# yyNoBug/VAE_segmentation

Measured on AMD Instinct MI355X. Metric: 3D train-step volumes/sec at 96^3 batch=2 (joint VAE+seg), higher is better.
Workload: dtype bf16; 1 GPU; configs[1]: 96^3 joint VAE+seg training step (joint_train), batch=2/GPU, bf16 activations + fp32 accumulate, SGD momentum 0.9, VAE frozen, HIP-graph replay; global_batch=2, parallelism=dp1, activation_recomputation=False, tail_in_graph=True, nranks=1, grad_exchange=none (1 rank)

## Files before the change

include/vaeseg.h:

```cpp
#ifndef VAESEG_H
#define VAESEG_H
#include <stddef.h>
#include <stdint.h>

#ifdef __cplusplus
extern "C" {
#endif

#define VS_VERSION 500

enum { VS_F32 = 0, VS_BF16 = 1, VS_F16 = 2, VS_F32X3 = 3  };
#ifndef VS_STAT_SLOTS
#define VS_STAT_SLOTS 4
#endif
enum { VS_OK = 0, VS_EINVAL = -1, VS_ESHAPE = -2, VS_EDTYPE = -3, VS_EWORKSPACE = -4, VS_EALIGN = -5 };

enum {
    VS_CONV_K3 = 0,
    VS_CONV_K2S2 = 1,
    VS_CONV_T2S2 = 2,
    VS_WGRAD_SLABS = 16,
    VS_CONV_UP = 3
};

enum {
    VS_PACK_ROWS_D0 = 0,
    VS_PACK_ROWS_D1_FLIP = 1,
    VS_PACK_SCATTER_D1 = 2
};

int vs_version(void);
int vs_stat_slots(void);
int vs_stat_interleaved(void);
const char* vs_strerror(int code);
int vs_get_deterministic(void);

int vs_up_supported(int cin, int cm, int co, int dtype);
int vs_up_compose_sizes(int cin, int cm, int co, size_t* out6);
int vs_up_compose(const float* w2, const float* b2, const float* w3, float* weff, void* img_fwd, void* img_bwd, int* taps_fwd, int* taps_bwd,
                  float* btab, int cin, int cm, int co, int dtype, void* stream);
int vs_up_conv_fwd(const void* x, const double* x_stats, const void* img_fwd, const int* taps_fwd, const float* btab, void* y, double* y_stats,
                   int n, int d, int h, int w, int cin, int co, int dtype, float eps, void* stream);
int vs_up_faces(const void* gy, double* G, int n, int fd, int fh, int fw, int co, int dtype, void* stream);
int vs_up_chain(const float* dweff27, const double* G, const float* w2, const float* b2, const float* w3, float* dw2, float* db2, float* dw3,
                int cin, int cm, int co, void* stream);
int vs_up_conv_bwd_data(const void* gy, const void* img_bwd, const int* taps_bwd, void* gx, const void* mask_x, const double* mask_stats,
                        double* sums, int n, int d, int h, int w, int co, int cin, int dtype, float eps, void* stream);

size_t vs_packed_weight_bytes(int rows, int c_pad, int ntaps, int dtype);
int vs_pack_weight(const float* src, void* dst, int d0, int d1, int ntaps, int c_pad, int form, int dtype, void* stream);

typedef struct vs_pack_desc {
    const float* src;
    void* dst;
    int d0, d1, ntaps, c_pad, form, dtype;
    int first_block;
    int pad_;
    long long total;
} vs_pack_desc;
int vs_pack_weight_multi(const vs_pack_desc* descs, int n_desc, int total_blocks, void* stream);

int vs_conv_gather_fwd(const void* x, const double* x_stats, const void* w_packed, const float* bias,
                       void* y, double* y_stats, int n, int d, int h, int w, int c_in, int m_out,
                       int kind, int dtype, float eps, void* stream);

int vs_conv_scatter_fwd(const void* x, const double* x_stats, const void* w_packed, const float* bias,
                        void* y, int n, int d, int h, int w, int c_in, int m_out, int dtype, float eps, void* stream);

int vs_conv_gather_bwd_data(const void* x, const void* w_packed, void* y, const void* mask_x, const double* mask_stats,
                            double* sums, int n, int d, int h, int w, int c_in, int m_out, int kind, int dtype, float eps,
                            void* stream);
int vs_conv_scatter_bwd_data(const void* x, const void* w_packed, void* y, const void* mask_x, const double* mask_stats,
                             double* sums, int n, int d, int h, int w, int c_in, int m_out, int dtype, float eps, void* stream);
int vs_conv_k3_fused_apply_supported(int n, int d, int h, int w, int c_in, int m_out, int lazy_input, int dtype);
int vs_conv_k3_bwd_data_wgrad_supported(int n, int d, int h, int w, int c_in, int m_out, int dtype);
int vs_conv_k3_bwd_data_wgrad_slabs(int n, int d, int h, int w);
int vs_conv_k3_bwd_data_wgrad(const void* g, const void* act_x, const double* act_stats, const double* act_sums, const void* w_packed, void* y,
                              const void* mask_x, const double* mask_stats, double* sums, float* slabs, int n, int d, int h, int w, int c_in,
                              int m_out, int dtype, float eps, void* stream);
int vs_conv_k3_softmax2_bwd_data(const float* prob, const float* gprob, const void* gprob_cl, const void* w_packed, void* y, const void* mask_x,
                                 const double* mask_stats, double* sums, float* slabs, double* bias_part, int n, int d, int h, int w, int dtype,
                                 float eps, float drop_p, unsigned long long drop_seed, void* stream);
typedef struct vs_config {
    int k3_small;
    int k3_tall;
    int k3_wgs_per_cu;
    int k3t_wgs_per_cu;
    int k3f_min_wgs;
    int mt_min_wgs;
    int f32_limbs;
    int g1_limbs;
    int k3x_ck;
    int k3x_toeplitz;
    int fuse_wgrad;
    int epilogue_apply;
    int chain;
    int k2s2_stream;
    int k2s8_wgs_per_cu;
    int up_wgs_per_cu;
    int up_rb;
    int wgrad_uber;
    int wgrad_mpack;
    int wgrad_swap;
    int wgrad_big;
    int wgrad_xcd;
    int k3_short_tiles;
    int wgrad_bias_fold;
    long long wgrad_wgs;
    long long wgrad_f32_tiles;
    long long wgrad_group_wgs;
    long long wgrad_big_min_voxels;
} vs_config;
int vs_config_bytes(void);
int vs_config_from_env(vs_config* c);
int vs_get_config(vs_config* out);
int vs_set_config(const vs_config* cfg);
int vs_conv_k3_bwd_data_applied_supported(int n, int d, int h, int w, int c_in, int m_out, int dtype);
int vs_conv_k3_bwd_data_applied(const void* x, const void* w_packed, void* y, const void* mask_x, const double* mask_stats, double* sums,
                                unsigned int* sync, unsigned int* fault, int n, int d, int h, int w, int c_in, int m_out, int dtype, float eps, void* stream);
int vs_conv_s2_bwd_data_applied_supported(int n, int d, int h, int w, int c_in, int m_out, int scatter, int dtype);
int vs_conv_s2_bwd_data_applied(const void* x, const void* w_packed, void* y, const void* mask_x, const double* mask_stats, double* sums, const void* add,
                                unsigned int* sync, unsigned int* fault, int n, int d, int h, int w, int c_in, int m_out, int scatter, int dtype, float eps,
                                void* stream);
typedef struct vs_chain_layer {
    const void* x;
    const double* x_stats;
    const void* w_packed;
    void* y;
    double* y_stats;
    const void* mask_x;
    const double* mask_stats;
    double* sums;
    int c_in, m_out;
    int apply;
    int reserved_;
} vs_chain_layer;
int vs_conv_k3_chain_supported(int n, int d, int h, int w, int c_max, int dtype);
long long vs_conv_k3_chain_sync_bytes(int n);
int vs_conv_k3_chain(const vs_chain_layer* layers, int n_layers, int backward, const void* add, unsigned int* sync, unsigned int* fault,
                     int n, int d, int h, int w, int dtype, float eps, void* stream);
int vs_conv_k3_f32_limbs(int d, int h, int w, int c_in);

int vs_conv_k3_bwd_data_fused_apply(const void* g, const void* act_x, const double* act_stats, const double* act_sums,
                                    const void* w_packed, void* y, const void* mask_x, const double* mask_stats, double* sums,
                                    void* dx_out, int n, int d, int h, int w, int c_in, int m_out, int dtype, float eps, void* stream);

int vs_conv_k3_softmax2_fwd(const void* x, const double* x_stats, const void* w_packed, const float* bias,
                            float* prob, int n, int d, int h, int w, int c_in, int dtype, float eps, void* stream);
int vs_conv_k3_softmax2_dropout_fwd(const void* x, const double* x_stats, const void* w_packed, const float* bias,
                                    float* prob, int n, int d, int h, int w, int c_in, int dtype, float eps, float drop_p,
                                    unsigned long long drop_seed, void* stream);
int vs_conv_k3_softmax2_cl_fwd(const void* x, const double* x_stats, const void* w_packed, const float* bias,
                               float* prob, void* prob_cl, int n, int d, int h, int w, int c_in, int dtype, float eps, float drop_p,
                               unsigned long long drop_seed, void* stream);

size_t vs_conv_wgrad_workspace_bytes(int n, int dp, int hp, int wp, int m_ch, int c_ch, int kind);
int vs_conv_wgrad(const void* p, const double* p_stats, const void* q, const double* q_stats, float* dw,
                  void* workspace, size_t workspace_bytes, int n, int dp, int hp, int wp, int m_ch, int c_ch,
                  int m_real, int c_real, int kind, int dtype, float eps, void* stream);
typedef struct vs_wgrad_desc {
    const void* p; const double* p_stats;
    const void* q; const double* q_stats;
    float* dw;
    const void* bias_g; float* db;
    long long bias_rows;
// ... 165 lines not shown
```

vae_segmentation_amd/modules.py:

```python
import torch
import torch.nn as nn

from . import ops

_DEFAULT_DTYPE = torch.float32


def set_default_kernel_dtype(dtype):
    global _DEFAULT_DTYPE
    if dtype not in ops.KERNEL_DTYPES:
        raise TypeError("kernel dtype must be torch.float32, torch.bfloat16 or torch.float16")
    _DEFAULT_DTYPE = dtype


def set_kernel_dtype(module, dtype):
    if dtype not in ops.KERNEL_DTYPES:
        raise TypeError("kernel dtype must be torch.float32, torch.bfloat16 or torch.float16")
    for m in module.modules():
        if hasattr(m, "kernel_dtype"):
            m.kernel_dtype = dtype
    return module


class Act:
# ... 217 lines not shown
        self.down4 = Down(f[3], f[4], norm_type=norm_type, soft=False)
        self.down5 = Down(f[4], f[5], norm_type=norm_type, soft=False)
        self.side = spatial // 32
        self.top_ch = f[5]
        flat = f[5] * self.side ** 3
        self.fc_mean = nn.Linear(flat, dim)
        self.fc_std = nn.Linear(flat, dim)
        self.fc2 = nn.Linear(dim, flat)
        self.up1 = Up(f[5], f[4], norm_type=norm_type, soft=False)
        self.up2 = Up(f[4], f[3], norm_type=norm_type, soft=False)
        self.up3 = Up(f[3], f[2], norm_type=norm_type, soft=False)
        self.up4 = Up(f[2], f[1], norm_type=norm_type, soft=False)
        self.up5 = Up(f[1], f[0], norm_type=norm_type, soft=False)
        self.out_block = nn.Conv3d(f[0], n_class, 3, padding=1)
        self.final = nn.Softmax(dim=1)
        self.n_class = n_class
        self.spatial = spatial
        self.kernel_dtype = _DEFAULT_DTYPE

    def forward(self, x, if_random=False, scale=1, mid_input=False, dropout=0.0, noise=None):
        ops._require_cuda(x)
        if not mid_input:
            if x.shape[-1] != self.spatial:
                raise ValueError("VAE built for spatial=%d got input side %d" % (self.spatial, x.shape[-1]))
            ops.stats_arena_begin(x.device)
            a = Act(ops.planar_input(x, self.kernel_dtype), None)
            a = self.in_block(a)
            if a.stats is not None:
                ops.mark_defer_apply(a.raw, self.in_block.conv[0])
            for blk in (self.down1, self.down2, self.down3, self.down4, self.down5):
                a = _run_block(blk, a)
                if blk is not self.down5 and a.stats is not None:
                    ops.mark_defer_apply(a.raw, blk.conv[1].conv[6])
            feat = ops.Materialize.apply(a.raw, a.stats, None, None)
            x_mean, x_std = ops.LinearCLPair.apply(feat, self.fc_mean.weight, self.fc_mean.bias, False,
                                                   self.fc_std.weight, self.fc_std.bias, True)
            if if_random:
                if noise is None:
                    noise = torch.randn(x_mean.shape, device=x_mean.device, dtype=torch.float32)
                z = ops.Reparam.apply(x_mean, x_std, noise.to(x_mean.device, torch.float32).contiguous(), scale)
            else:
                z = x_mean
        else:
            ops.stats_arena_begin(x.device)
            z = x
        h = ops.LinearToCL.apply(z, self.fc2.weight, self.fc2.bias, self.top_ch, self.side, self.kernel_dtype)
        a = Act(h, None)
        for blk in (self.up1, self.up2, self.up3, self.up4, self.up5):
            a = _dropout(_run_block(blk, a), dropout)
            if a.stats is not None:
                ops.mark_defer_apply(a.raw, blk.conv[1].conv[6])
        recon = ops.ConvK3Softmax.apply(a.raw, a.stats, self.out_block.weight, self.out_block.bias)
        if not mid_input:
            return recon, x_mean, x_std
        return recon


class Segmentation(nn.Module):

    def __init__(self, n_channels, n_class, norm_type=2, n_fmaps=[8, 16, 32, 64, 128, 256]):
        super().__init__()
        _check_n_class(n_class)
        f = list(n_fmaps)
        self.in_block = Conv(n_channels, f[0], norm_type=norm_type, soft=False)
        self.down1 = Down(f[0], f[1], norm_type=norm_type, soft=False)
        self.down2 = Down(f[1], f[2], norm_type=norm_type, soft=False)
        self.down3 = Down(f[2], f[3], norm_type=norm_type, soft=False)
        self.down4 = Down(f[3], f[4], norm_type=norm_type, soft=False)
        self.up2 = Up(f[4], f[3], norm_type=norm_type, soft=False)
        self.up3 = Up(f[3], f[2], norm_type=norm_type, soft=False)
        self.up4 = Up(f[2], f[1], norm_type=norm_type, soft=False)
        self.up5 = Up(f[1], f[0], norm_type=norm_type, soft=False)
        self.out_block = nn.Conv3d(f[0], n_class, 3, padding=1)
        self.final = nn.Softmax(dim=1)
        self.n_class = n_class
        self.kernel_dtype = _DEFAULT_DTYPE

    def forward(self, data_dict, in_key, out_key, dropout=0.0):
        x = data_dict[in_key]
        ops._require_cuda(x)
        if any(s % 16 for s in x.shape[2:]):
            raise ValueError("Segmentation needs spatial sizes that are multiples of 16, got %s" % (tuple(x.shape[2:]),))
        ops.stats_arena_begin(x.device)
        a = Act(ops.PackPlanar.apply(x, self.kernel_dtype), None)
        x1 = self.in_block(a)
        x2 = _run_block(self.down1, x1)
        x3 = _run_block(self.down2, x2)
        x4 = _run_block(self.down3, x3)
        x5 = _run_block(self.down4, x4)
        u = _dropout(_run_block(self.up2, x5), dropout)
        u = _run_block(self.up3, u)
        u = _dropout(Act(ops.Materialize.apply(u.raw, u.stats, x3.raw, x3.stats, True), None), dropout)
        u = _run_block(self.up4, u)
        u = _dropout(Act(ops.Materialize.apply(u.raw, u.stats, x2.raw, x2.stats, True), None), dropout)
        u = _dropout(_run_block(self.up5, u), dropout)
        if u.stats is not None:
            ops.mark_defer_apply(u.raw, self.up5.conv[1].conv[6])
        if dropout:
            data_dict[out_key] = ops.out_block_softmax(u.raw, u.stats, self.out_block.weight, self.out_block.bias,
                                                       float(dropout), ops.next_dropout_seed())
        else:
            data_dict[out_key] = ops.out_block_softmax(u.raw, u.stats, self.out_block.weight, self.out_block.bias)
        return data_dict


class Joint(nn.Module):

    def __init__(self, models, vae_forward_scale=0.0, vae_decoder_dropout=0.0, seg_dropout=0.0):
        super().__init__()
        self.Seg = models[0]
        self.Vae = models[1]
        self.vae_forward_scale = vae_forward_scale
        self.vae_decoder_dropout = vae_decoder_dropout
        self.seg_dropout = seg_dropout

    def forward(self, data_dict, in_key, out_key, out_key_recon, dropout=False):
        with ops.arena_scope(data_dict[in_key].device):
            if dropout:
                data_dict = self.Seg(data_dict, in_key, out_key, dropout=self.seg_dropout)
                data_dict[out_key_recon], _, _ = self.Vae(data_dict[out_key], if_random=False, scale=self.vae_forward_scale,
                                                          dropout=self.vae_decoder_dropout)
            else:
                data_dict = self.Seg(data_dict, in_key, out_key)
                data_dict[out_key_recon], data_dict["mean"], data_dict["std"] = self.Vae(
                    data_dict[out_key], if_random=False, scale=self.vae_forward_scale)
        return data_dict


def _linear(x2d, fc, relu):
    return ops.LinearCL.apply(x2d.contiguous().view(x2d.shape[0], 1, 1, 1, x2d.shape[1]), fc.weight, fc.bias, relu)


class Encoder(nn.Module):

    def __init__(self, n_channels, dim, norm_type=2, n_fmaps=[8, 16, 32, 64, 128, 256], soft=False, spatial=128):
        super().__init__()
        if spatial % 32 or spatial < 64:
            raise ValueError("spatial must be a multiple of 32 and >= 64")
        f = list(n_fmaps)
        self.in_block = Conv(n_channels, f[0], norm_type=norm_type, soft=False)
        self.down1 = Down(f[0], f[1], norm_type=norm_type, soft=False)
        self.down2 = Down(f[1], f[2], norm_type=norm_type, soft=False)
        self.down3 = Down(f[2], f[3], norm_type=norm_type, soft=False)
        self.down4 = Down(f[3], f[4], norm_type=norm_type, soft=False)
        self.down5 = Down(f[4], f[5], norm_type=norm_type, soft=False)
        self.fc1 = nn.Linear(f[5] * (spatial // 32) ** 3, 1024)
        self.fc2 = nn.Linear(1024, 128)
        self.fc_mean = nn.Linear(128, dim)
        self.spatial = spatial
        self.kernel_dtype = _DEFAULT_DTYPE

    def forward(self, x):
        ops._require_cuda(x)
        if x.shape[-1] != self.spatial:
            raise ValueError("Encoder built for spatial=%d got input side %d" % (self.spatial, x.shape[-1]))
        ops.stats_arena_begin(x.device)
        a = Act(ops.PackPlanar.apply(x.contiguous(), self.kernel_dtype), None)
        a = self.in_block(a)
        for blk in (self.down1, self.down2, self.down3, self.down4, self.down5):
            a = blk(a)
        feat = ops.Materialize.apply(a.raw, a.stats, None, None)
        h = ops.LinearCL.apply(feat, self.fc1.weight, self.fc1.bias, True)
        h = _linear(h, self.fc2, True)
        return torch.sigmoid(_linear(h, self.fc_mean, False))


class Fusion(nn.Module):

# ... 86 lines not shown
```

vae_segmentation_amd/ops.py:

```python
import ctypes as _ctypes
import os
import weakref as _weakref

import torch

from . import _lib
from ._lib import (VS_BF16, VS_CONV_K2S2, VS_CONV_K3, VS_CONV_UP, VS_F16, VS_F32, VS_PACK_ROWS_D0, VS_PACK_ROWS_D1_FLIP,
                   VS_PACK_SCATTER_D1, check, lib)

_DT_TORCH = {VS_F32: torch.float32, VS_BF16: torch.bfloat16, VS_F16: torch.float16}
_DT_VS = {v: k for k, v in _DT_TORCH.items()}
KERNEL_DTYPES = tuple(_DT_VS)
VS_F32X3 = 3
F32X3 = "f32x3"
_DT_TORCH[VS_F32X3] = F32X3
_DT_VS[F32X3] = VS_F32X3
_F32_LIMBS = bool(lib.vs_conv_k3_f32_limbs(96, 96, 96, 8))


def k3_pack_dtype(x):
    if x.dtype == torch.float32 and lib.vs_conv_k3_f32_limbs(x.shape[1], x.shape[2], x.shape[3], x.shape[4]):
        return F32X3
    return x.dtype

# ... 876 lines not shown
    tname = _tname(x)
    with _timed("in_relu_bwd_reduce_kernel<%s>" % tname, 2 * x.numel() * _esize(x), 4.0 * x.numel(), str(tuple(x.shape))):
        check(lib.vs_instnorm_relu_bwd_reduce(g.data_ptr(), x.data_ptr(), xs.data_ptr(), sums.data_ptr(), n, voxels, c, dt,
                                              EPS_IN, _stream()), "instnorm_relu_bwd_reduce")
    gx = g if inplace else torch.empty_like(g)
    with _timed("in_relu_bwd_apply_kernel<%s>" % tname, 3 * x.numel() * _esize(x), 6.0 * x.numel(), str(tuple(x.shape))):
        check(lib.vs_instnorm_relu_bwd_apply(g.data_ptr(), x.data_ptr(), xs.data_ptr(), sums.data_ptr(), gx.data_ptr(), n,
                                             voxels, c, dt, EPS_IN, _stream()), "instnorm_relu_bwd_apply")
    return gx


def _contig(t):
    return t if t.is_contiguous() else t.contiguous()


class ConvK3(torch.autograd.Function):

    @staticmethod
    def forward(ctx, x, xs, weight, bias, live_bias=False):
        _require_cuda(x, weight)
        cout, cin = weight.shape[0], weight.shape[1]
        wp = pack_weight_cached(weight, VS_PACK_ROWS_D0, x.shape[-1], k3_pack_dtype(x))
        ctx.live_bias = bool(live_bias) and bias is not None
        b_use = bias if ctx.live_bias else None
        if b_use is not None and cout < cpad(cout):
            b_use = torch.nn.functional.pad(b_use.detach().float(), (0, cpad(cout) - cout))
        y, ys = conv_gather(x, xs, wp, b_use, cpad(cout), VS_CONV_K3, True, real_channels=(cin, cout))
        ctx.save_for_backward(x, xs, weight)
        ctx.has_bias = bias is not None
        ctx.bias_ref = bias
        ctx.defer = bool(getattr(x, "_vs_defer_apply", False)) and xs is not None
        if ctx.needs_input_grad[2]:
            _count_use(weight)
        ctx.mark_non_differentiable(ys)
        ctx.set_materialize_grads(False)
        return y, ys

    @staticmethod
    def backward(ctx, gy, _gys):
        x, xs, weight = ctx.saved_tensors
        if gy is None:
            return None, None, None, None, None
        gy = _contig(gy)
        cout, cin = weight.shape[0], weight.shape[1]
        gx = gw = gb = None
        lazy = _take_lazy(gy)
        if lazy is not None and not (ctx.needs_input_grad[0] and _fa_supported(gy, x, xs is not None)):
            gy, lazy = apply_lazy(gy, lazy), None
        if ctx.needs_input_grad[0]:
            wpb = pack_weight_cached(weight, VS_PACK_ROWS_D1_FLIP, gy.shape[-1], k3_pack_dtype(gy))
            want_gb0 = ctx.has_bias and ctx.needs_input_grad[3] and ctx.live_bias
            if xs is not None and ctx.needs_input_grad[2] and not want_gb0 and _wgrad_fusable(gy, x, weight):
                gx, gw = conv_bwd_data_lazy(gy, wpb, x, xs, VS_CONV_K3, real_channels=(cout, cin), defer=ctx.defer, lazy=lazy,
                                            fuse_wgrad=(weight, cout, cin))
                gb = _dead_bias_grad(ctx.bias_ref, ctx.bias_ref.shape[0], x.device) if ctx.has_bias and ctx.needs_input_grad[3] else None
                return gx, None, gw, gb, None
            if lazy is not None and xs is not None:
                gx, gy = conv_bwd_data_lazy(gy, wpb, x, xs, VS_CONV_K3, real_channels=(cout, cin), defer=ctx.defer, lazy=lazy,
                                            want_dx=ctx.needs_input_grad[2])
            elif lazy is not None:
                ax, axs, asums = lazy
                gx = torch.empty_like(x)
                dx = torch.empty_like(gy) if ctx.needs_input_grad[2] else None
                n_, d_, h_, w_, c_ = gy.shape
                check(lib.vs_conv_k3_bwd_data_fused_apply(gy.data_ptr(), ax.data_ptr(), axs.data_ptr(), asums.data_ptr(), wpb.data_ptr(), gx.data_ptr(),
                                                          None, None, None, _p(dx), n_, d_, h_, w_, c_, x.shape[-1], vs_dtype(x), EPS_IN, _stream()),
                      "conv_k3_bwd_data_fused_apply")
                gy = dx
            elif xs is not None:
                gx = conv_bwd_data_lazy(gy, wpb, x, xs, VS_CONV_K3, real_channels=(cout, cin), defer=ctx.defer)
            else:
                gx, _ = conv_gather(gy, None, wpb, None, x.shape[-1], VS_CONV_K3, False, real_channels=(cout, cin))
        want_gb = ctx.has_bias and ctx.needs_input_grad[3]
        if ctx.needs_input_grad[2]:
            gw, gb = _side_grads(weight, (gy, x, xs), (gy, None, x, xs, cout, cin, VS_CONV_K3),
                                 (gy, cout) if want_gb and ctx.live_bias else None, ctx.bias_ref if ctx.live_bias else None)
        elif want_gb and ctx.live_bias:
            gb = bias_grad(gy, cout)
        if want_gb and not ctx.live_bias:
            gb = _dead_bias_grad(ctx.bias_ref, ctx.bias_ref.shape[0], x.device)
        return gx, None, gw, gb, None


CHAIN = os.environ.get("VS_CHAIN", "1") != "0"


class ChainLayer(_ct.Structure):
    _fields_ = [("x", _ct.c_void_p), ("x_stats", _ct.c_void_p), ("w_packed", _ct.c_void_p), ("y", _ct.c_void_p), ("y_stats", _ct.c_void_p),
                ("mask_x", _ct.c_void_p), ("mask_stats", _ct.c_void_p), ("sums", _ct.c_void_p), ("c_in", _ct.c_int), ("m_out", _ct.c_int),
                ("apply", _ct.c_int), ("reserved_", _ct.c_int)]


_CHAIN_FAULT = {}


def _chain_fault_word(device):
    key = torch.device(device)
    t = _CHAIN_FAULT.get(key)
    if t is None:
        if torch.cuda.is_current_stream_capturing():
            raise RuntimeError("the chain fault word must exist before a capture starts: run the step eagerly once (GraphedStep warms up)")
        t = _CHAIN_FAULT[key] = torch.zeros(32, dtype=torch.int32, device=key)
    return t


def chain_fault():
    for dev, t in _CHAIN_FAULT.items():
        if int(t[0].item()) != 0:
            raise _lib.VaesegError("a chain kernel on %s gave up a bounded wait (workgroups of one sample not co-resident): results invalid; set VS_CHAIN=0" % (dev,))


def device_is_shared(shared=True):
    global CHAIN, EPILOGUE_APPLY
    on = 0 if shared else 1
    set_config(chain=on, epilogue_apply=on)
    CHAIN = EPILOGUE_APPLY = not shared


def _chain_sync(n, device):
    cnt = lib.vs_conv_k3_chain_sync_bytes(n) // 8
    buf = _new_stats(1, cnt + 16, device, width=1).view(-1)
    off = ((-buf.data_ptr()) % 128) // 8
    return buf[off:off + cnt]


def chain_ok(x, xs, convs):
    if not CHAIN or len(convs) < 2 or len(convs) > 3 or x.dtype not in KERNEL_DTYPES:
        return False
    if getattr(x, "_vs_defer_apply", False):
        return False
    if any(tuple(c.weight.shape[2:]) != (3, 3, 3) for c in convs):
        return False
    n, d, h, w, c = x.shape
    cmax = max([c] + [cpad(cv.weight.shape[0]) for cv in convs])
    return bool(lib.vs_conv_k3_chain_supported(n, d, h, w, cmax, vs_dtype(x)))


class ConvK3Chain(torch.autograd.Function):

    @staticmethod
    def forward(ctx, x, xs, *params):
        _require_cuda(x)
        nl = len(params) // 2
        weights, biases = params[0::2], params[1::2]
        n, d, h, w, _ = x.shape
        layers = (ChainLayer * nl)()
        cur, curs, outs, keep = x, xs, [], []
        nb = fl = 0.0
        for l in range(nl):
            wt = weights[l]
            m = cpad(wt.shape[0])
            wp = pack_weight_cached(wt, VS_PACK_ROWS_D0, cur.shape[-1], k3_pack_dtype(cur))
            y = torch.empty((n, d, h, w, m), dtype=x.dtype, device=x.device)
            ys = _new_stats(n, m, x.device)
            layers[l] = ChainLayer(cur.data_ptr(), _p(curs), wp.data_ptr(), y.data_ptr(), ys.data_ptr(), None, None, None, cur.shape[-1], m, 0, 0)
            keep.append(wp)
            nb += (cur.numel() + y.numel() + wt.numel()) * _esize(x)
            fl += 2.0 * n * d * h * w * 27 * wt.shape[0] * wt.shape[1]
            outs.append((y, ys))
            cur, curs = y, ys
            if ctx.needs_input_grad[2 + 2 * l]:
                _count_use(wt)
        sync = _chain_sync(n, x.device)
        with _timed("k3_chain<%s,fwd,%d>" % (_tname(x), nl), nb, fl, "x%s" % (tuple(x.shape),)):
            check(lib.vs_conv_k3_chain(_ct.addressof(layers), nl, 0, None, sync.data_ptr(), _chain_fault_word(x.device).data_ptr(), n, d, h, w,
                                       vs_dtype(x), EPS_IN, _stream()), "conv_k3_chain (forward)")
# ... 1277 lines not shown
```

vae_segmentation_amd/profiling.py:

```python
import torch

from . import ops

LAST_LAUNCHES = []
HBM_PEAK_GBS = 8000.0
MFMA_PEAK_TFLOPS = {"bf16": 2500.0, "fp16": 2500.0, "f32": 2500.0 / 6.0}


LAST_EVENT_OVERHEAD_US = 0.0


def _spin(us, stream):
    from tools import probe
    probe.check(probe.lib.vs_spin(int(us), stream), "spin")


ops.PROFILE_SPIN[0] = _spin


def event_bracket_overhead_us(trials=24, spin_us=20):
    stream = torch.cuda.current_stream().cuda_stream
    over = []
    for _ in range(trials):
        _spin(ops.PROFILE_PRIME_US, stream)
# ... 8 lines not shown


def collect(fwd_bwd, params, steps=2):
    for p in params:
        p.grad = None
    fwd_bwd()
    torch.cuda.synchronize()
    ops.PROFILE = []
    try:
        for _ in range(steps):
            for p in params:
                p.grad = None
            fwd_bwd()
        torch.cuda.synchronize()
        recs = ops.PROFILE
    finally:
        ops.PROFILE = None
    agg = {}
    global LAST_LAUNCHES, LAST_EVENT_OVERHEAD_US
    LAST_EVENT_OVERHEAD_US = event_bracket_overhead_us()
    dur = lambda e0, e1: max(e0.elapsed_time(e1) - LAST_EVENT_OVERHEAD_US * 1e-3, 1e-4)
    LAST_LAUNCHES = sorted(((dur(e0, e1), kid, det, nb, fl) for kid, nb, fl, det, e0, e1 in recs), reverse=True)
    for kid, nb, fl, det, e0, e1 in recs:
        a = agg.setdefault(kid, {"launches": 0, "ms": 0.0, "bytes": 0.0, "flops": 0.0})
        a["launches"] += 1
        a["ms"] += dur(e0, e1)
        a["bytes"] += nb
        a["flops"] += fl
    for a in agg.values():
        for k in ("launches", "ms", "bytes", "flops"):
            a[k] = a[k] / steps
    return agg


def sources_sha():
    import glob
    import hashlib
    import os
    root = os.path.dirname(os.path.dirname(os.path.abspath(__file__)))
    h = hashlib.sha256()
    files = sorted(glob.glob(os.path.join(root, "vae_segmentation_amd", "csrc", "*.hip")) + glob.glob(os.path.join(root, "vae_segmentation_amd", "csrc", "*.h")) +
                   glob.glob(os.path.join(root, "vae_segmentation_amd", "csrc", "*.inc")) + [os.path.join(root, "include", "vaeseg.h")])
    for f in files:
        h.update(os.path.basename(f).encode())
        h.update(open(f, "rb").read())
    return h.hexdigest()[:16]


def traffic_is_stale(path=None):
    import json
    try:
        table = json.load(open(path or _traffic_path()))
    except Exception:
        return None
    return table.get("_sources_sha16") != sources_sha()


def _traffic_path():
    import glob
    import os
    cands = sorted(glob.glob(os.path.join(os.path.dirname(os.path.dirname(os.path.abspath(__file__))), "profiles", "r*_hbm_traffic.json")))
    return cands[-1] if cands else ""


def measured_step_traffic(path=None):
    import json
    try:
        table = json.load(open(path or _traffic_path()))
    except Exception:
        return None
    if "_step_total_bytes" in table:
        return table["_step_total_bytes"]
    try:
        tot = float(sum(rec["hbm_bytes_per_launch"] * rec.get("launches_per_step", 0) for rec in table.values() if isinstance(rec, dict)))
    except Exception:
        return None
    return tot if tot > 0 else None


FAMILIES = (
    ("conv3x3x3, C>=32 levels (k3b<32,..>, k3s)", lambda k: k.startswith("k3b_kernel<32") or k.startswith("k3s_kernel") or k.startswith("chain")),
    ("conv3x3x3, 16-channel layers (k3b<16|8,..>)", lambda k: k.startswith("k3b_kernel<16") or k.startswith("k3b_kernel<8")),
    ("conv3x3x3, 8-channel full-resolution layers (k3t; k3tw = backward-data + the layer's weight gradient)", lambda k: k.startswith("k3t_kernel") or k.startswith("k3tw_kernel")),
    ("conv3x3x3, fp32 kernels (k3_kernel<float>)", lambda k: k.startswith("k3_kernel")),
    ("composed Up heads: transposed conv + 3x3x3 as one operator (k4t, k4g)", lambda k: k.startswith("k4t_kernel") or k.startswith("k4g_kernel")),
    ("stride-2 / transposed convs (g1)", lambda k: k.startswith("g1_kernel")),
    ("weight gradients (grouped)", lambda k: k.startswith("wgrad_multi") or k.startswith("g3")),
    ("InstanceNorm+ReLU backward apply", lambda k: k.startswith("in_relu_bwd")),
)


def kernel_families(fwd_bwd, params, dtype, steps=2):
    agg = collect(fwd_bwd, params, steps)
    peak_tf = MFMA_PEAK_TFLOPS["f32" if dtype == "fp32" else dtype]
    fam = {}
    for kid, a in agg.items():
        name = next((n for n, pred in FAMILIES if pred(kid)), "other timed launches")
        f = fam.setdefault(name, {"launches_per_step": 0.0, "ms_per_step": 0.0, "bytes": 0.0, "flops": 0.0, "kernels": []})
        f["launches_per_step"] += a["launches"]
        f["ms_per_step"] += a["ms"]
        f["bytes"] += a["bytes"]
        f["flops"] += a["flops"]
        f["kernels"].append(kid)
    out = []
    for name, f in sorted(fam.items(), key=lambda kv: -kv[1]["ms_per_step"]):
        sec = f["ms_per_step"] * 1e-3
        hbm_bound = f["bytes"] / (HBM_PEAK_GBS * 1e9) >= f["flops"] / (peak_tf * 1e12)
        ach = f["bytes"] / sec / 1e9 if hbm_bound else f["flops"] / sec / 1e12
        peak = HBM_PEAK_GBS if hbm_bound else peak_tf
        out.append({"family": name, "bound": "hbm" if hbm_bound else "mfma", "achieved": round(ach, 2), "peak": peak,
                    "unit": "GB/s" if hbm_bound else "TFLOP/s", "frac": round(ach / peak, 4),
                    "launches_per_step": round(f["launches_per_step"], 1), "ms_per_step": round(f["ms_per_step"], 4),
                    "avg_launch_us": round(1e3 * f["ms_per_step"] / max(f["launches_per_step"], 1e-9), 2),
                    "algorithmic_bytes_per_step": f["bytes"], "algorithmic_flops_per_step": f["flops"],
                    "kernels": sorted(set(f["kernels"]))})
    return {"method": "HIP events around every launch of real eager passes, bracket overhead %.2f us subtracted" % LAST_EVENT_OVERHEAD_US,
            "timed_ms_per_step": round(sum(f["ms_per_step"] for f in fam.values()), 4), "entries": out}


def _norm_name(name):
    name = name.replace("void ", "").split("(")[0]
    return name.replace(" ", "")


def measured_traffic(kid, path=None):
    import json
    import os
    path = path or _traffic_path()
    try:
        table = json.load(open(path))
    except Exception:
        return None
    want = _norm_name(kid)
    for name, rec in table.items():
        if _norm_name(name) == want:
            return rec["hbm_bytes_per_launch"]
    return None


def dominant_kernel_roofline(fwd_bwd, params, dtype, steps=2, kernel=None):
    agg = collect(fwd_bwd, params, steps)
    if not agg:
        return None
    kid = kernel if kernel in agg else max(agg, key=lambda k: agg[k]["ms"])
    a = agg[kid]
    sec = a["ms"] * 1e-3
    mfma_peak = MFMA_PEAK_TFLOPS["f32"] if "float" in kid else MFMA_PEAK_TFLOPS["bf16"]
    t_hbm = a["bytes"] / (HBM_PEAK_GBS * 1e9)
    t_mfma = a["flops"] / (mfma_peak * 1e12)
    total_ms = sum(v["ms"] for v in agg.values())
    if t_hbm >= t_mfma:
        ach, peak, unit, bound = a["bytes"] / sec / 1e9, HBM_PEAK_GBS, "GB/s", "hbm"
    else:
        ach, peak, unit, bound = a["flops"] / sec / 1e12, mfma_peak, "TFLOP/s", "mfma"
    top = sorted(agg.items(), key=lambda kv: -kv[1]["ms"])[:6]

    def bound_of(v):
        peak_tf = MFMA_PEAK_TFLOPS["f32"] if "float" in v[0] else MFMA_PEAK_TFLOPS["bf16"]
        s = v[1]["ms"] * 1e-3
        if v[1]["bytes"] / (HBM_PEAK_GBS * 1e9) >= v[1]["flops"] / (peak_tf * 1e12):
            return {"kernel": v[0], "bound": "hbm", "achieved": round(v[1]["bytes"] / s / 1e9, 1), "peak": HBM_PEAK_GBS, "unit": "GB/s",
                    "frac": round(v[1]["bytes"] / s / 1e9 / HBM_PEAK_GBS, 4), "launches_per_step": v[1]["launches"],
                    "avg_launch_us": round(1e3 * v[1]["ms"] / v[1]["launches"], 2), "traffic": measured_traffic(v[0])}
        return {"kernel": v[0], "bound": "mfma", "achieved": round(v[1]["flops"] / s / 1e12, 2), "peak": peak_tf, "unit": "TFLOP/s",
                "frac": round(v[1]["flops"] / s / 1e12 / peak_tf, 4), "launches_per_step": v[1]["launches"],
                "avg_launch_us": round(1e3 * v[1]["ms"] / v[1]["launches"], 2), "traffic": measured_traffic(v[0])}
# ... 7 lines not shown
```

Before: 897.0 volumes/s.

## Add planar single-channel input conv kernels fusing pack, conv, stats and wgrad

Adds dedicated HIP kernels for the first 3x3x3 conv, which has 1 input channel and 8 output channels. The forward reads the fp32 planar image directly, skipping the separate pack-to-channels-last pass, and computes the InstanceNorm statistics in the same kernel. The backward applies the lazy InstanceNorm+ReLU backward and computes the weight gradient with MFMA in one pass, emitting slabs that are reduced through the grouped wgrad path. The new path adds code complexity and is used only when the input needs no gradient and the dtype is bf16 or fp16.

After: 898.0 volumes/s, median of 6. No clear change (+0.1%).

```diff
diff --git a/include/vaeseg.h b/include/vaeseg.h
--- a/include/vaeseg.h
+++ b/include/vaeseg.h
@@ -81,6 +81,11 @@
 int vs_conv_k3_softmax2_bwd_data(const float* prob, const float* gprob, const void* gprob_cl, const void* w_packed, void* y, const void* mask_x,
                                  const double* mask_stats, double* sums, float* slabs, double* bias_part, int n, int d, int h, int w, int dtype,
                                  float eps, float drop_p, unsigned long long drop_seed, void* stream);
+int vs_conv_in_planar_supported(int n, int d, int h, int w, int c_in, int m_out, int dtype);
+int vs_conv_in_planar_slabs(int n, int d, int h, int w);
+int vs_conv_in_planar_fwd(const float* img, const float* weight, void* y, double* y_stats, int n, int d, int h, int w, int dtype, float eps, void* stream);
+int vs_conv_in_planar_bwd_weight(const void* g, const void* act_x, const double* act_stats, const double* act_sums, const float* img, float* slabs,
+                                 int n, int d, int h, int w, int dtype, float eps, void* stream);
 typedef struct vs_config {
     int k3_small;
     int k3_tall;
diff --git a/vae_segmentation_amd/csrc/in_planar.hip b/vae_segmentation_amd/csrc/in_planar.hip
--- /dev/null
+++ b/vae_segmentation_amd/csrc/in_planar.hip
@@ -0,0 +1,351 @@
+#include "common.h"
+
+namespace {
+
+constexpr int TZ = 4, TY = 8, TX = 32;
+constexpr int HZ = TZ + 2, HY = TY + 2, HX = TX + 2;
+constexpr int HV = HZ * HY * HX;
+constexpr int NLD = (HV + 255) / 256;
+constexpr int TVOX = TZ * TY * TX;
+constexpr int INP_MAX_N = 32;
+
+struct InpParams {
+    const float* img;
+    const float* w;
+    void* y;
+    double* y_stats;
+    const void* g;
+    const double* sums;
+    float* slabs;
+    int N, D, H, W;
+    int txn, tyn, tiles_per_sample, total_tiles;
+    double inv_count;
+    float eps;
+};
+
+struct Coord { int n, z0, y0, x0; };
+__device__ __forceinline__ Coord inp_tile(const InpParams& p, int t) {
+    Coord c;
+    c.n = t / p.tiles_per_sample;
+    const int tl = t - c.n * p.tiles_per_sample;
+    const int per_z = p.txn * p.tyn;
+    const int tz = tl / per_z, r = tl - tz * per_z, ty = r / p.txn;
+    c.z0 = tz * TZ; c.y0 = ty * TY; c.x0 = (r - ty * p.txn) * TX;
+    return c;
+}
+
+template <typename T>
+__device__ __forceinline__ void inp_load_halo(const InpParams& p, const Coord& c, int tid, float (&v)[NLD]) {
+#pragma unroll
+    for (int b = 0; b < NLD; ++b) {
+        const int hv = tid + b * 256;
+        const int hx = hv % HX, hy = (hv / HX) % HY, hz = hv / (HX * HY);
+        const int gz = c.z0 - 1 + hz, gy = c.y0 - 1 + hy, gx = c.x0 - 1 + hx;
+        const bool ok = hv < HV && (unsigned)gz < (unsigned)p.D && (unsigned)gy < (unsigned)p.H && (unsigned)gx < (unsigned)p.W;
+        float f = 0.f;
+        if (ok) f = p.img[(((size_t)c.n * p.D + gz) * p.H + gy) * p.W + gx];
+        v[b] = ET<T>::rnd(f);
+    }
+}
+
+template <typename T>
+__global__ __launch_bounds__(256) void inp_fwd_kernel(const InpParams p) {
+    __shared__ float s_img[NLD * 256];
+    __shared__ __attribute__((aligned(16))) float s_w[27 * 8];
+    __shared__ float s_red[4][8][2];
+    const int tid = threadIdx.x, lane = tid & 63, wave = tid >> 6;
+    const int x = tid & 31, y = tid >> 5;
+    const int G = (int)gridDim.x;
+    for (int i = tid; i < 27 * 8; i += 256) s_w[i] = ET<T>::rnd(p.w[(i & 7) * 27 + (i >> 3)]);
+
+    int t = (int)blockIdx.x;
+    Coord cur = inp_tile(p, t < p.total_tiles ? t : 0), nxt = cur;
+    float pre[NLD];
+    if (t < p.total_tiles) inp_load_halo<T>(p, cur, tid, pre);
+    float ssum[8], ssq[8];
+#pragma unroll
+    for (int c = 0; c < 8; ++c) { ssum[c] = 0.f; ssq[c] = 0.f; }
+
+    for (; t < p.total_tiles; t += G) {
+#pragma unroll
+        for (int b = 0; b < NLD; ++b) s_img[tid + b * 256] = pre[b];
+        __syncthreads();
+        const bool more = t + G < p.total_tiles;
+        nxt = inp_tile(p, more ? t + G : t);
+        if (more) inp_load_halo<T>(p, nxt, tid, pre);
+
+        f32x2 acc[TZ][4];
+#pragma unroll
+        for (int oz = 0; oz < TZ; ++oz)
+#pragma unroll
+            for (int c = 0; c < 4; ++c) acc[oz][c] = f32x2{0.f, 0.f};
+#pragma unroll 1
+        for (int dd = 0; dd < 9; ++dd) {
+            const int dy = dd / 3, dx = dd - 3 * dy;
+            const float* const col = s_img + (y + dy) * HX + x + dx;
+            float in[HZ];
+#pragma unroll
+            for (int zz = 0; zz < HZ; ++zz) in[zz] = col[zz * HY * HX];
+#pragma unroll
+            for (int dz = 0; dz < 3; ++dz) {
+                const float* wt = s_w + (dz * 9 + dd) * 8;
+                const f32x4 wa = *(const f32x4*)wt, wb = *(const f32x4*)(wt + 4);
+                const f32x2 w2[4] = {f32x2{wa[0], wa[1]}, f32x2{wa[2], wa[3]}, f32x2{wb[0], wb[1]}, f32x2{wb[2], wb[3]}};
+#pragma unroll
+                for (int oz = 0; oz < TZ; ++oz) {
+                    const f32x2 v = f32x2{in[oz + dz], in[oz + dz]};
+#pragma unroll
+                    for (int c = 0; c < 4; ++c) acc[oz][c] = v * w2[c] + acc[oz][c];
+                }
+            }
+        }
+
+        const int n = cur.n, oy = cur.y0 + y, ox = cur.x0 + x;
+#pragma unroll
+        for (int oz = 0; oz < TZ; ++oz) {
+            const int gz = cur.z0 + oz;
+            const bool valid = gz < p.D && oy < p.H && ox < p.W;
+            u32x4 pk;
+#pragma unroll
+            for (int c = 0; c < 4; ++c) pk[c] = H16<T>::pack2(acc[oz][c]);
+            if (valid) {
+                *(u32x4*)((T*)p.y + ((((size_t)n * p.D + gz) * p.H + oy) * p.W + ox) * 8) = pk;
+#pragma unroll
+                for (int c = 0; c < 4; ++c) {
+                    const float lo = H16<T>::lo(pk[c]), hi = H16<T>::hi(pk[c]);
+                    ssum[2 * c] += lo; ssq[2 * c] += lo * lo;
+                    ssum[2 * c + 1] += hi; ssq[2 * c + 1] += hi * hi;
+                }
+            }
+        }
+        const bool flush = !more || nxt.n != n;
+        if (flush) {
+#pragma unroll
+            for (int c = 0; c < 8; ++c) {
+                const float s = wave_sum(ssum[c]), q = wave_sum(ssq[c]);
+                if (lane == 0) { s_red[wave][c][0] = s; s_red[wave][c][1] = q; }
+                ssum[c] = 0.f; ssq[c] = 0.f;
+            }
+            __syncthreads();
+            if (tid < 16) {
+                const int ch = tid >> 1, st = tid & 1;
+                const double tot = (double)s_red[0][ch][st] + (double)s_red[1][ch][st] + (double)s_red[2][ch][st] + (double)s_red[3][ch][st];
+                stat_add(p.y_stats, (size_t)n * 8 + ch, (size_t)p.N * 8, st, tot);
+            }
+        }
+        cur = nxt;
+        __syncthreads();
+    }
+}
+
+template <typename T, bool LAZY>
+__global__ __launch_bounds__(256) void inp_bwd_kernel(const InpParams p) {
+    __shared__ __attribute__((aligned(16))) T s_img[3][HZ][HY][TX];
+    __shared__ __attribute__((aligned(16))) T s_dy[8][TVOX];
+    __shared__ float s_tab[4][INP_MAX_N * 8];
+    __shared__ float s_part[4][2][8][16];
+    const int tid = threadIdx.x, lane = tid & 63, wave = tid >> 6, col = lane & 15, q = lane >> 4;
+    const int x = tid & 31, y = tid >> 5;
+    const int G = (int)gridDim.x;
+    const T* const gp = (const T*)p.g;
+    const T* const xp = (const T*)p.y;
+
+    if constexpr (LAZY) {
+        for (int i = tid; i < p.N * 8; i += 256) {
+            float m, r;
+            stats_to_mean_rstd(p.y_stats, (size_t)i, (size_t)p.N * 8, p.inv_count, p.eps, m, r);
+            double sv[2];
+            stat_load(p.sums, (size_t)i, (size_t)p.N * 8, sv);
+            s_tab[0][i] = m; s_tab[1][i] = r;
+            s_tab[2][i] = (float)(sv[0] * p.inv_count);
+            s_tab[3][i] = (float)(sv[1] * p.inv_count);
+        }
+    }
+    int boff[2];
+    bool bok[2];
+#pragma unroll
+    for (int h = 0; h < 2; ++h) {
+        const int tap = 16 * h + col;
+        const int dz = tap / 9, dy = (tap / 3) % 3, dx = tap % 3;
+        bok[h] = tap < 27;
+        boff[h] = bok[h] ? ((dx * HZ + dz) * HY + dy) * TX + q * 8 : 0;
+    }
+    f32x4 acc[2] = {f32x4{0.f, 0.f, 0.f, 0.f}, f32x4{0.f, 0.f, 0.f, 0.f}};
+
+    int t = (int)blockIdx.x;
+    Coord cur = inp_tile(p, t < p.total_tiles ? t : 0), nxt = cur;
+    float pre[NLD];
+    u32x4 gq[TZ], xq[TZ];
+    auto load_gx = [&](const Coord& c) {
+#pragma unroll
+        for (int oz = 0; oz < TZ; ++oz) {
+            const int gz = c.z0 + oz, gy = c.y0 + y, gx = c.x0 + x;
+            const bool ok = gz < p.D && gy < p.H && gx < p.W;
+            const size_t e = ok ? ((((size_t)c.n * p.D + gz) * p.H + gy) * p.W + gx) * 8 : 0;
+            gq[oz] = *(const u32x4*)(gp + e);
+            if constexpr (LAZY) xq[oz] = *(const u32x4*)(xp + e);
+        }
+    };
+    if (t < p.total_tiles) { inp_load_halo<T>(p, cur, tid, pre); load_gx(cur); }
+    __syncthreads();
+
+    for (; t < p.total_tiles; t += G) {
+#pragma unroll
+        for (int b = 0; b < NLD; ++b) {
+            const int hv = tid + b * 256;
+            const int hx = hv % HX, hy = (hv / HX) % HY, hz = hv / (HX * HY);
+            T hvT;
+            ET<T>::st(&hvT, pre[b]);
+            if (hv < HV) {
+#pragma unroll
+                for (int dx = 0; dx < 3; ++dx)
+                    if (hx - dx >= 0 && hx - dx < TX) s_img[dx][hz][hy][hx - dx] = hvT;
+            }
+        }
+        {
+            float tm[8], tr[8], ta[8], tb[8];
+            if constexpr (LAZY) {
+#pragma unroll
+                for (int c = 0; c < 8; ++c) {
+                    tm[c] = s_tab[0][cur.n * 8 + c]; tr[c] = s_tab[1][cur.n * 8 + c];
+                    ta[c] = s_tab[2][cur.n * 8 + c]; tb[c] = s_tab[3][cur.n * 8 + c];
+                }
+            }
+#pragma unroll
+            for (int oz = 0; oz < TZ; ++oz) {
+                const bool ok = cur.z0 + oz < p.D && cur.y0 + y < p.H && cur.x0 + x < p.W;
+                float fg[8], o[8];
+                frag_unpack(gq[oz], fg, (T*)nullptr);
+                if constexpr (LAZY) {
+                    float fx[8];
+                    frag_unpack(xq[oz], fx, (T*)nullptr);
+#pragma unroll
+                    for (int c = 0; c < 8; ++c) o[c] = vs_in_bwd_apply1(fg[c], fx[c], tm[c], tr[c], ta[c], tb[c]);
+                } else {
+#pragma unroll
+                    for (int c = 0; c < 8; ++c) o[c] = fg[c];
+                }
+                const int v = (oz * TY + y) * TX + x;
+#pragma unroll
+                for (int c = 0; c < 8; ++c) ET<T>::st(&s_dy[c][v], ok ? o[c] : 0.f);
+            }
+        }
+        __syncthreads();
+        const bool more = t + G < p.total_tiles;
+        nxt = inp_tile(p, more ? t + G : t);
+        if (more) { inp_load_halo<T>(p, nxt, tid, pre); load_gx(nxt); }
+
+        const u32x4 zero4 = u32x4{0u, 0u, 0u, 0u};
+#pragma unroll
+        for (int i = 0; i < 8; ++i) {
+            const int ks = wave * 8 + i, kz = ks >> 3, ky = ks & 7;
+            const u32x4 a = col < 8 ? *(const u32x4*)(&s_dy[col][ks * TX + q * 8]) : zero4;
+            const T* const ib = &s_img[0][0][0][0] + (kz * HY + ky) * TX;
+#pragma unroll
+            for (int h = 0; h < 2; ++h) {
+                const u32x4 bfr = bok[h] ? *(const u32x4*)(ib + boff[h]) : zero4;
+                acc[h] = mfma16(a, bfr, acc[h], (T*)nullptr);
+            }
+        }
+        cur = nxt;
+        __syncthreads();
+    }
+
+    if (q < 2) {
+#pragma unroll
+        for (int h = 0; h < 2; ++h)
+#pragma unroll
+            for (int i = 0; i < 4; ++i) s_part[wave][h][4 * q + i][col] = acc[h][i];
+    }
+    __syncthreads();
+    if (tid < 27 * 8) {
+        const int tap = tid >> 3, co = tid & 7;
+        const float tot = ((s_part[0][tap >> 4][co][tap & 15] + s_part[1][tap >> 4][co][tap & 15]) + s_part[2][tap >> 4][co][tap & 15]) + s_part[3][tap >> 4][co][tap & 15];
+        p.slabs[(size_t)blockIdx.x * 1728 + (26 - tap) * 64 + co] = tot;
+    }
+}
+
+int inp_cu_count() {
+    static int known[64] = {0};
+    int dev = 0, cus = 0;
+    if (hipGetDevice(&dev) != hipSuccess) return 0;
+    if (dev >= 0 && dev < 64 && known[dev] > 0) return known[dev];
+    if (hipDeviceGetAttribute(&cus, hipDeviceAttributeMultiprocessorCount, dev) != hipSuccess || cus <= 0) return 0;
+    if (dev >= 0 && dev < 64) known[dev] = cus;
+    return cus;
+}
+
+int inp_grid(long long tiles) {
+    const int cus = inp_cu_count();
+    if (cus <= 0 || tiles <= 0) return 0;
+    const long long cap = 2ll * cus;
+    const long long rounds = (tiles + cap - 1) / cap;
+    return (int)((tiles + rounds - 1) / rounds);
+}
+
+bool inp_fill(InpParams& p, int n, int d, int h, int w) {
+    p.N = n; p.D = d; p.H = h; p.W = w;
+    p.txn = (w + TX - 1) / TX;
+    p.tyn = (h + TY - 1) / TY;
+    const long long tps = (long long)((d + TZ - 1) / TZ) * p.tyn * p.txn;
+    if (tps * n >= 2147483647ll) return false;
+    p.tiles_per_sample = (int)tps;
+    p.total_tiles = (int)(tps * n);
+    p.inv_count = 1.0 / ((double)d * h * w);
+    return true;
+}
+
+}
+
+extern "C" int vs_conv_in_planar_supported(int n, int d, int h, int w, int c_in, int m_out, int dtype) {
+    if (dtype != VS_BF16 && dtype != VS_F16) return 0;
+    if (c_in != 1 || m_out != 8) return 0;
+    if (n <= 0 || n > INP_MAX_N || d <= 0 || h <= 0 || w <= 0) return 0;
+    InpParams p{};
+    return inp_fill(p, n, d, h, w) ? 1 : 0;
+}
+
+extern "C" int vs_conv_in_planar_slabs(int n, int d, int h, int w) {
+    InpParams p{};
+    if (n <= 0 || d <= 0 || h <= 0 || w <= 0 || !inp_fill(p, n, d, h, w)) return 0;
+    return inp_grid(p.total_tiles);
+}
+
+extern "C" int vs_conv_in_planar_fwd(const float* img, const float* weight, void* y, double* y_stats, int n, int d, int h, int w, int dtype, float eps,
+                                     void* stream) {
+    if (!img || !weight || !y || !y_stats) return VS_EINVAL;
+    if (!vs_conv_in_planar_supported(n, d, h, w, 1, 8, dtype)) return VS_ESHAPE;
+    if ((uintptr_t)y & 15) return VS_EINVAL;
+    InpParams p{};
+    inp_fill(p, n, d, h, w);
+    p.img = img; p.w = weight; p.y = y; p.y_stats = y_stats; p.eps = eps;
+    const int grid = inp_grid(p.total_tiles);
+    if (grid <= 0) return VS_EINVAL;
+    if (dtype == VS_BF16) hipLaunchKernelGGL(inp_fwd_kernel<unsigned short>, dim3(grid), dim3(256), 0, (hipStream_t)stream, p);
+    else hipLaunchKernelGGL(inp_fwd_kernel<vs_half>, dim3(grid), dim3(256), 0, (hipStream_t)stream, p);
+    VS_CHECK_LAUNCH();
+    return VS_OK;
+}
+
+extern "C" int vs_conv_in_planar_bwd_weight(const void* g, const void* act_x, const double* act_stats, const double* act_sums, const float* img, float* slabs,
+                                            int n, int d, int h, int w, int dtype, float eps, void* stream) {
+    if (!g || !img || !slabs) return VS_EINVAL;
+    const bool lazy = act_x != nullptr;
+    if (lazy != (act_stats != nullptr) || lazy != (act_sums != nullptr)) return VS_EINVAL;
+    if (!vs_conv_in_planar_supported(n, d, h, w, 1, 8, dtype)) return VS_ESHAPE;
+    if (((uintptr_t)g & 15) || ((uintptr_t)act_x & 15)) return VS_EINVAL;
+    InpParams p{};
+    inp_fill(p, n, d, h, w);
+    p.img = img; p.g = g; p.y = const_cast<void*>(act_x); p.y_stats = const_cast<double*>(act_stats); p.sums = act_sums; p.slabs = slabs; p.eps = eps;
+    const int grid = inp_grid(p.total_tiles);
+    if (grid <= 0) return VS_EINVAL;
+    dispatch_t(dtype, [&](auto* tag) {
+        using T = TAG_T(tag);
+        if constexpr (sizeof(T) == 2) {
+            if (lazy) hipLaunchKernelGGL((inp_bwd_kernel<T, true>), dim3(grid), dim3(256), 0, (hipStream_t)stream, p);
+            else hipLaunchKernelGGL((inp_bwd_kernel<T, false>), dim3(grid), dim3(256), 0, (hipStream_t)stream, p);
+        }
+    });
+    VS_CHECK_LAUNCH();
+    return VS_OK;
+}
diff --git a/vae_segmentation_amd/modules.py b/vae_segmentation_amd/modules.py
--- a/vae_segmentation_amd/modules.py
+++ b/vae_segmentation_amd/modules.py
@@ -323,8 +323,12 @@
         if any(s % 16 for s in x.shape[2:]):
             raise ValueError("Segmentation needs spatial sizes that are multiples of 16, got %s" % (tuple(x.shape[2:]),))
         ops.stats_arena_begin(x.device)
-        a = Act(ops.PackPlanar.apply(x, self.kernel_dtype), None)
-        x1 = self.in_block(a)
+        c0 = self.in_block.conv
+        if isinstance(c0[1], nn.InstanceNorm3d) and isinstance(c0[2], nn.ReLU) and ops.planar_in_ok(x, c0[0], self.kernel_dtype):
+            y, ys = ops.ConvInPlanar.apply(x, c0[0].weight, c0[0].bias, self.kernel_dtype)
+            x1 = Act(ops.mark_defer_apply(y, c0[0]), ys)
+        else:
+            x1 = self.in_block(Act(ops.PackPlanar.apply(x, self.kernel_dtype), None))
         x2 = _run_block(self.down1, x1)
         x3 = _run_block(self.down2, x2)
         x4 = _run_block(self.down3, x3)
diff --git a/vae_segmentation_amd/ops.py b/vae_segmentation_amd/ops.py
--- a/vae_segmentation_amd/ops.py
+++ b/vae_segmentation_amd/ops.py
@@ -982,6 +982,85 @@
         return gx, None, gw, gb, None
 
 
+PLANAR_IN = os.environ.get("VS_PLANAR_IN", "1") != "0"
+
+
+def planar_in_supported(x, weight, dtype):
+    if not PLANAR_IN or dtype == torch.float32 or x.dim() != 5 or weight.dim() != 5 or tuple(weight.shape[2:]) != (3, 3, 3):
+        return False
+    if not hasattr(lib, "vs_conv_in_planar_supported"):
+        return False
+    n, _, d, h, w = x.shape
+    return bool(lib.vs_conv_in_planar_supported(n, d, h, w, weight.shape[1], weight.shape[0], vs_of(dtype)))
+
+
+def planar_in_ok(x, conv, dtype):
+    wt = conv.weight
+    if x.requires_grad and torch.is_grad_enabled():
+        return False
+    if not (FUSE_WGRAD and _GROUP["enabled"] and wt.is_leaf and wt.dtype == torch.float32 and not _has_hooks(wt)):
+        return False
+    return planar_in_supported(x, wt, dtype)
+
+
+def _slabs_reduce_now(slabs, nslabs, m_real, c_real, gw, dtype):
+    d = WgradDesc(slabs.data_ptr(), None, None, None, gw.data_ptr(), None, None, 0, 0, 0, nslabs, 0, 0, 0, 8, 8, m_real, c_real, VS_WGRAD_SLABS, 0)
+    arr = (WgradDesc * 1)(d)
+    ws = torch.empty(256, dtype=torch.uint8, device=slabs.device)
+    check(lib.vs_conv_wgrad_multi(_ct.addressof(arr), 1, ws.data_ptr(), 256, vs_of(dtype), EPS_IN, _stream()), "conv_wgrad_multi")
+
+
+class ConvInPlanar(torch.autograd.Function):
+
+    @staticmethod
+    def forward(ctx, x, weight, bias, dtype):
+        _require_cuda(x, weight)
+        x = _contig(x.float())
+        n, _, d, h, w = x.shape
+        wt = _contig(weight.detach())
+        y = torch.empty((n, d, h, w, 8), dtype=dtype, device=x.device)
+        ys = _new_stats(n, 8, x.device)
+        with _timed("inp_fwd_kernel<%s>" % _tname(y), x.numel() * 4 + y.numel() * 2, 2.0 * x.numel() * 27 * 8, "x%s->m8" % (tuple(x.shape),)):
+            check(lib.vs_conv_in_planar_fwd(x.data_ptr(), wt.data_ptr(), y.data_ptr(), ys.data_ptr(), n, d, h, w, vs_dtype(y), EPS_IN, _stream()),
+                  "conv_in_planar_fwd")
+        ctx.save_for_backward(x, weight)
+        ctx.has_bias = bias is not None
+        ctx.bias_ref = bias
+        if ctx.needs_input_grad[1]:
+            _count_use(weight)
+        ctx.mark_non_differentiable(ys)
+        ctx.set_materialize_grads(False)
+        return y, ys
+
+    @staticmethod
+    def backward(ctx, gy, _gys):
+        x, weight = ctx.saved_tensors
+        if gy is None:
+            return None, None, None, None
+        gy = _contig(gy)
+        lazy = _take_lazy(gy)
+        gw = gb = None
+        if ctx.needs_input_grad[1]:
+            n, d, h, w, _ = gy.shape
+            ax, axs, asums = lazy if lazy is not None else (None, None, None)
+            nslabs = lib.vs_conv_in_planar_slabs(n, d, h, w)
+            slabs = torch.empty(nslabs * 1728, dtype=torch.float32, device=gy.device)
+            kid = "inp_bwd_kernel<%s,%s>" % (_tname(gy), "true" if lazy is not None else "false")
+            with _timed(kid, (2 if lazy is not None else 1) * gy.numel() * 2 + x.numel() * 4, 2.0 * x.numel() * 27 * 8, "gy%s" % (tuple(gy.shape),)):
+                check(lib.vs_conv_in_planar_bwd_weight(gy.data_ptr(), _p(ax), _p(axs), _p(asums), x.data_ptr(), slabs.data_ptr(), n, d, h, w, vs_dtype(gy),
+                                                       EPS_IN, _stream()), "conv_in_planar_bwd_weight")
+            deferrable = (_GROUP["enabled"] and weight.is_leaf and weight.grad is None and not _has_hooks(weight) and not torch.is_grad_enabled()
+                          and getattr(weight, "_vs_use", None) == [_USE_EPOCH[0], 1] and _GROUP["slots"].get(id(weight)) is None)
+            if deferrable:
+                gw = _group_submit_slabs(weight, slabs, nslabs, 8, 1, (gy, x) + (() if lazy is None else tuple(lazy)))
+            else:
+                gw = torch.empty(weight.shape, dtype=torch.float32, device=gy.device)
+                _slabs_reduce_now(slabs, nslabs, 8, 1, gw, gy.dtype)
+        if ctx.has_bias and ctx.needs_input_grad[2]:
+            gb = _dead_bias_grad(ctx.bias_ref, ctx.bias_ref.shape[0], x.device)
+        return None, gw, gb, None
+
+
 CHAIN = os.environ.get("VS_CHAIN", "1") != "0"
 
 
diff --git a/vae_segmentation_amd/profiling.py b/vae_segmentation_amd/profiling.py
--- a/vae_segmentation_amd/profiling.py
+++ b/vae_segmentation_amd/profiling.py
@@ -114,6 +114,7 @@
     ("conv3x3x3, C>=32 levels (k3b<32,..>, k3s)", lambda k: k.startswith("k3b_kernel<32") or k.startswith("k3s_kernel") or k.startswith("chain")),
     ("conv3x3x3, 16-channel layers (k3b<16|8,..>)", lambda k: k.startswith("k3b_kernel<16") or k.startswith("k3b_kernel<8")),
     ("conv3x3x3, 8-channel full-resolution layers (k3t; k3tw = backward-data + the layer's weight gradient)", lambda k: k.startswith("k3t_kernel") or k.startswith("k3tw_kernel")),
+    ("in_block from the planar image (inp_fwd; inp_bwd = IN-backward apply + weight gradient)", lambda k: k.startswith("inp_fwd_kernel") or k.startswith("inp_bwd_kernel")),
     ("conv3x3x3, fp32 kernels (k3_kernel<float>)", lambda k: k.startswith("k3_kernel")),
     ("composed Up heads: transposed conv + 3x3x3 as one operator (k4t, k4g)", lambda k: k.startswith("k4t_kernel") or k.startswith("k4g_kernel")),
     ("stride-2 / transposed convs (g1)", lambda k: k.startswith("g1_kernel")),
```
